# Ajax0564/VyomAI

Hardware: AMD Instinct MI355X
Metric: training tokens/sec (12L d=768 seq=512 GPT-style decoder, CLM) (higher is better)
Workload: dtype bf16; 1 GPU; configs[1]: GPT-style Decoder 12L d=768 h=12 RoPE vocab 50265, CLM training B=32/GPU seq=512, AdamW, bf16 kernels + fp32 masters; global_batch=32, seq_len=512, parallelism=dp1, attention=none, weights=deterministic recipe (vyomai_amd.recipe)

## Files before the change

### include/vyom_hip.h

```cpp
#ifndef VYOM_HIP_H
#define VYOM_HIP_H

#include <stdint.h>

#ifdef __cplusplus
extern "C" {
#endif

typedef enum { VY_F32 = 0, VY_BF16 = 1 } vy_dtype;

typedef enum {
  VY_OK = 0,
  VY_ERR_ARG = -1,
  VY_ERR_UNSUPPORTED = -2,
  VY_ERR_LAUNCH = -3
} vy_status;

typedef enum {
  VY_ACT_NONE = 0, VY_ACT_GELU_ERF = 1, VY_ACT_GELU_TANH = 2,
  VY_ACT_SILU = 3, VY_ACT_TANH = 4, VY_ACT_SIGMOID = 5, VY_ACT_RELU6 = 6, VY_ACT_LEAKY_RELU = 7
} vy_act;
#define VY_ACT_SAVE_DERIV 0x100

enum {
// ... 190 lines not shown
int vy_linear_dropout_fwd(const void* x, int64_t ldx, const void* w, int64_t ldw, const void* bias,
                          const void* residual, int64_t ldr, void* y, int64_t ldy, int64_t M, int64_t N,
                          int64_t K, float p_drop, uint64_t seed, uint64_t offset, int dtype, void* stream);
int vy_dropout(const void* x, int64_t ldx, void* y, int64_t ldy, int64_t M, int64_t N, float p_drop,
               uint64_t seed, uint64_t offset, int dtype, void* stream);

int vy_act_bwd(const void* dy, int64_t lddy, const void* pre, int64_t ldpre, void* dx, int64_t lddx,
               int64_t M, int64_t N, int act, int dtype, void* stream);

int vy_xent_fwd(const void* logits, int64_t ld, const int64_t* labels, int64_t ignore_index, float* lse,
                float* loss_sum, float* count, int64_t M, int64_t V, int32_t* err_flag, int dtype, void* stream);
int vy_xent_bwd(void* logits, int64_t ld, const int64_t* labels, int64_t ignore_index, const float* lse,
                const float* gscale, const float* count, int64_t M, int64_t V, int dtype, void* stream);
int vy_xent_fused(void* logits, int64_t ld, const int64_t* labels, int64_t ignore_index, float* lse,
                  float* loss_sum, const float* count, const float* gscale, int64_t M, int64_t V,
                  int32_t* err_flag, int dtype, void* stream);
int vy_xent_sample_fwd(const void* logits, int64_t ld, const int64_t* labels, int64_t ignore_index, float* lse,
                       float* loss_sum, float* count, int64_t* sampled, float inv_temperature, uint64_t seed,
                       uint64_t offset, int64_t M, int64_t V, int32_t* err_flag, int dtype, void* stream);
int vy_xent_sample_fused(void* logits, int64_t ld, const int64_t* labels, int64_t ignore_index, float* lse,
                         float* loss_sum, const float* count, const float* gscale, int64_t* sampled,
                         float inv_temperature, uint64_t seed, uint64_t offset, int64_t M, int64_t V,
                         int32_t* err_flag, int dtype, void* stream);
int vy_gumbel_noise(float* out, int64_t ld, int64_t M, int64_t V, uint64_t seed, uint64_t offset, void* stream);

int vy_bce_head_fwd(const void* h, int64_t ldh, const void* w, const void* b, float* z, const float* target,
                    const uint8_t* live, float* loss_sum, int64_t M, int64_t d, int dtype, void* stream);
int vy_bce_head_bwd(const void* h, int64_t ldh, const void* w, const float* z, const float* target,
                    const uint8_t* live, const float* gscale, const float* count, void* dh, int64_t lddh, float* dw,
                    float* db, int accumulate, int64_t M, int64_t d, int dtype, void* stream);

int vy_mlm_mask(const int64_t* ids, int64_t n, const int64_t* special_ids, int32_t n_special, float fraction,
                int64_t mask_id, int64_t vocab, int64_t ignore_index, uint64_t seed, uint64_t offset,
                int64_t* masked_ids, int64_t* labels, uint8_t* masked, void* stream);


int vy_logprob_fwd(const void* logits, int64_t ld, const int64_t* labels, const float* weight, float* lse,
                   float* logp, int64_t M, int64_t V, int32_t* err_flag, int dtype, void* stream);
int vy_logprob_bwd(void* logits, int64_t ld, const int64_t* labels, const float* weight, const float* lse,
                   int64_t M, int64_t V, int dtype, void* stream);
int vy_logprob_fused(void* logits, int64_t ld, const int64_t* labels, const float* weight, float* lse,
                     float* logp, int64_t M, int64_t V, int32_t* err_flag, int dtype, void* stream);

int vy_embedding_fwd(const void* table, int64_t ldt, const int64_t* ids, void* out, int64_t ldo,
                     int64_t M, int64_t d, int64_t V, int32_t* err_flag, int dtype, void* stream);
int vy_embedding_bwd(const void* dout, int64_t lddo, const int64_t* ids, float* dw, int64_t lddw,
// ... 126 lines not shown
```

### vyomai_amd/_lib.py

```python
from __future__ import annotations

import ctypes as C
import os
from typing import Optional

_HERE = os.path.dirname(os.path.abspath(__file__))
LIB_PATH = os.environ.get("VY_LIB_PATH") or os.path.join(_HERE, "lib", "libvyom_hip.so")

VY_F32, VY_BF16 = 0, 1
ACT_NONE, ACT_GELU_ERF, ACT_GELU_TANH = 0, 1, 2
ACT_SILU, ACT_TANH, ACT_SIGMOID, ACT_RELU6, ACT_LEAKY_RELU = 3, 4, 5, 6, 7
ACT_SAVE_DERIV = 0x100
LORA_EPI_ACT, LORA_EPI_DROP_RES, LORA_EPI_MUL = 0, 1, 2
MASK_NONE, MASK_CAUSAL, MASK_KEYPAD, MASK_ADDITIVE = 0, 1, 2, 4

_p, _i64, _i, _f, _u64 = C.c_void_p, C.c_int64, C.c_int, C.c_float, C.c_uint64

PROTOTYPES = {
    "vy_linear_fwd": [_p, _i64, _p, _i64, _p, _p, _i64, _p, _i64, _p, _i64, _i64, _i64, _i, _i, _p],
    "vy_qkv_rope_fwd": [_p, _i64, _p, _i64, _p, _p, _p, _i64,
                        _p, _i64, _i64, _i64, _p, _i64, _i64, _i64, _p, _i64, _i64, _i64,
                        _i64, _i64, _i64, _i, _i, _i, _i, _p],
    "vy_attn_fwd": [_p, _i64, _i64, _i64, _p, _i64, _i64, _i64, _p, _i64, _i64, _i64,
                    _p, _i64, _i64, _p, _i, _i64, _p, _i64, _p, _i64, _i64,
# ... 23 lines not shown
                           _i64, _i64, _i, _i, _i, _i, _p],
    "vy_qknorm_bwd": [_p, _i64, _p, _i64, _p, _p, _f, _p, _p, _f, _p, _i64, _i, _i, _i, _i, _p],
    "vy_rope_fwd": [_p, _i64, _i64, _i64, _p, _p, _i64, _i64, _i, _i64, _i, _i, _i, _p],
    "vy_linear_dgrad": [_p, _i64, _p, _i64, _p, _i64, _i, _p, _i64, _p, _i64, _p, _i64, _i64, _i64, _i64, _i, _p],
    "vy_linear_wgrad": [_p, _i64, _p, _i64, _p, _i64, _p, _f, _p, _i64, _i64, _i64, _i, _p],
    "vy_linear_wgrad_grouped": [_p, _i, _i, _p],
    "vy_linear_wgrad_grouped_cs": [_p, _i, _p, _i, _i, _p],
    "vy_linear_wgrad_grouped_opt": [_p, _i, _p, _i, _p, _i, _p, _i, _p],
    "vy_layernorm_bwd_partial": [_p, _i64, _p, _i64, _p, _p, _p, _p, _i64, _p, _i64, _i64, _i, _p],
    "vy_layernorm_bwd": [_p, _i64, _p, _i64, _p, _p, _p, _p, _i64, _p, _p, _f, _p, _i64, _i64, _i, _p],
    "vy_attn_bwd": [_p, _i64, _i64, _i64, _p, _i64, _i64, _i64, _p, _i64, _i64, _i64,
                    _p, _p, _i64, _i64, _p, _p,
                    _p, _i64, _i64, _i64, _p, _i64, _i64, _i64, _p, _i64, _i64, _i64,
                    _i, _i64, _p, _i64, _p, _p, _i64, _i64, _i, _i, _i64, _i64, _i, _f, _i, _p],
    "vy_adamw_step": [_p, _p, _p, _p, _p, _i64, _f, _f, _f, _f, _f, _i64, _f, _p, _p],
    "vy_adamw_step_gated": [_p, _p, _p, _p, _p, _i64, _f, _f, _f, _f, _f, _i64, _f, _p, _p, _p],
    "vy_sumsq": [_p, _i64, _p, _p, _p],
    "vy_linear_dropout_fwd": [_p, _i64, _p, _i64, _p, _p, _i64, _p, _i64, _i64, _i64, _i64, _f, _u64, _u64, _i, _p],
    "vy_dropout": [_p, _i64, _p, _i64, _i64, _i64, _f, _u64, _u64, _i, _p],
    "vy_act_bwd": [_p, _i64, _p, _i64, _p, _i64, _i64, _i64, _i, _i, _p],
    "vy_xent_fwd": [_p, _i64, _p, _i64, _p, _p, _p, _i64, _i64, _p, _i, _p],
    "vy_xent_bwd": [_p, _i64, _p, _i64, _p, _p, _p, _i64, _i64, _i, _p],
    "vy_xent_fused": [_p, _i64, _p, _i64, _p, _p, _p, _p, _i64, _i64, _p, _i, _p],
    "vy_xent_sample_fwd": [_p, _i64, _p, _i64, _p, _p, _p, _p, _f, _u64, _u64, _i64, _i64, _p, _i, _p],
    "vy_xent_sample_fused": [_p, _i64, _p, _i64, _p, _p, _p, _p, _p, _f, _u64, _u64, _i64, _i64, _p, _i, _p],
    "vy_gumbel_noise": [_p, _i64, _i64, _i64, _u64, _u64, _p],
    "vy_bce_head_fwd": [_p, _i64, _p, _p, _p, _p, _p, _p, _i64, _i64, _i, _p],
    "vy_bce_head_bwd": [_p, _i64, _p, _p, _p, _p, _p, _p, _p, _i64, _p, _p, _i, _i64, _i64, _i, _p],
    "vy_mlm_mask": [_p, _i64, _p, _i, _f, _i64, _i64, _i64, _u64, _u64, _p, _p, _p, _p],
    "vy_logprob_fwd": [_p, _i64, _p, _p, _p, _p, _i64, _i64, _p, _i, _p],
    "vy_logprob_bwd": [_p, _i64, _p, _p, _p, _i64, _i64, _i, _p],
    "vy_logprob_fused": [_p, _i64, _p, _p, _p, _p, _i64, _i64, _p, _i, _p],
    "vy_transpose_batched": [_p, _i, _i, _i, _p],
    "vy_embedding_fwd": [_p, _i64, _p, _p, _i64, _i64, _i64, _i64, _p, _i, _p],
    "vy_embedding_bwd": [_p, _i64, _p, _p, _i64, _i64, _i64, _i64, _i64, _i, _p],
    "vy_transpose": [_p, _i64, _p, _i64, _i64, _i64, _i, _p],
    "vy_greedy_step": [_p, _i64, _i64, _i64, _i, _p, _i64, _i64, _p, _i64, _p, _i, _p, _p, _p],
    "vy_sampling_probs": [_p, _i64, _i64, _i64, _i, _f, _i, _f, _p, _i64, _p],
    "vy_sample_rows": [_p, _i64, _i64, _i64, _i, _p, _p, _p, _p, _p, _p, _p],
    "vy_spec_verify": [_p, _i64, _i64, _p, _i64, _i64, _i64, _i64, _i64, _i, _p, _p, _p, _p, _p, _p, _p, _p, _p, _p, _p],
    "vy_lora_shrink": [_p, _i64, _p, _p, _i64, _p, _i64, _i64, _i64, _i64, _i64, _i, _p],
    "vy_lora_expand": [_p, _i64, _p, _i64, _p, _p, _p, _i64, _i64, _i64, _i64, _i64, _i64, _i64, _i, _p],
    "vy_lora_expand_epi": [_p, _i64, _p, _i64, _p, _i64, _p, _i64, _p, _i64, _p, _p, _p, _i64, _i64, _i64, _i64, _i64,
                           _i64, _i64, _i, _i, _f, _u64, _u64, _i, _p],
    "vy_cls_head_fwd": [_p, _i64, _p, _p, _p, _p, _p, _p, _p, _i64, _i64, _i64, _i, _p],
    "vy_cls_head_bwd": [_p, _i64, _p, _p, _p, _p, _p, _p, _i, _i64, _i64, _i64, _i64, _i, _p],
# ... 102 lines not shown
```

### vyomai_amd/autograd_train.py

```python
from __future__ import annotations

import os

import weakref
from typing import NamedTuple, Optional

import torch

from . import _lib, ops
from ._lib import ACT_GELU_ERF, ACT_NONE, VyomHipError
from .autograd import gated_mlp
from .layers.attention import _shadow
from .layers.mask import AttnMask
from .layers.positional_embeddings import resolve_freqs

BF16 = torch.bfloat16


WEIGHT_EPOCH = [0]


class _WtRegistry:

    def __init__(self) -> None:
# ... 581 lines not shown
    dt = n.dtype
    V = w.shape[0]
    ld = _row_stride(V)
    buf = torch.empty((n.numel() // n.shape[-1], ld), dtype=dt, device=n.device)
    if zero_pad and ld != V:
        buf[:, V:].zero_()
    logits = buf[:, :V]
    ops.linear(n.view(buf.shape[0], -1), _shadow(w, dt), None if bias is None else _shadow(bias, dt), out=logits)
    return buf, logits


def _rehome(x, ld, dtype, reuse=False):
    V = x.shape[-1]
    if reuse and x.stride(-1) == 1 and x.stride(-2) == ld and x.dtype == dtype:
        buf = torch.as_strided(x, (*x.shape[:-1], ld), x.stride())
        if ld != V:
            buf[..., V:].zero_()
        return buf
    buf = torch.zeros((*x.shape[:-1], ld), dtype=dtype, device=x.device)
    buf[..., :V] = x
    return buf


def _shifted_labels(labels, ignore_index, dev):
    shifted = torch.full(labels.shape, ignore_index, dtype=torch.long, device=dev)
    shifted[:, :-1] = labels[:, 1:]
    return shifted.view(-1)


def _xent_forward(logits, shifted, ignore_index, err_flag=None, in_place=True, sample=None):
    V = logits.shape[1]
    dev = logits.device
    lse = torch.empty(logits.shape[0], dtype=torch.float32, device=dev)
    acc = torch.zeros(2, dtype=torch.float32, device=dev)
    fused = in_place and V <= 65536 and logits.dtype == BF16
    if fused:
        acc[1] = ((shifted != ignore_index) & (shifted >= 0) & (shifted < V)).sum()
        if sample is None:
            ops.xent_fused_(logits, shifted, ignore_index, lse, acc[0:1], acc[1:2], _one(dev), err_flag)
        else:
            ops.xent_sample_fused_(logits, shifted, ignore_index, lse, acc[0:1], acc[1:2], _one(dev), *sample, err_flag)
    elif sample is None:
        ops.xent_fwd(logits, shifted, ignore_index, lse, acc[0:1], acc[1:2], err_flag)
    else:
        ops.xent_sample_fwd(logits, shifted, ignore_index, lse, acc[0:1], acc[1:2], *sample, err_flag)
    return acc[0] / acc[1].clamp_min(1.0), lse, acc, fused


def _xent_backward(logits, shifted, ignore_index, lse, acc, fused, gout):
    gs = gout.detach().to(torch.float32).reshape(1).contiguous()
    if fused:
        return gs
    ops.xent_bwd_(logits, shifted, ignore_index, lse, gs, acc[1:2])
    return None


class LMHeadFn(torch.autograd.Function):

    @staticmethod
    def forward(ctx, hidden, wd, bd, ln_w, ln_b, wv, bias, eps):
        _require_bf16(hidden)
        dt = hidden.dtype
        pre, g, n, mean, rstd = _head_transform(hidden, wd, bd, ln_w, ln_b, eps)
        V = wv.shape[0]
        ld = _row_stride(V)
        buf = torch.zeros((*hidden.shape[:-1], ld), dtype=dt, device=hidden.device)
        logits = buf[..., :V]
        ops.linear(n, _shadow(wv, dt), _shadow(bias, dt), out=logits)
        ctx.save_for_backward(hidden, pre, g, n, mean, rstd)
        ctx.params = (wd, bd, ln_w, ln_b, wv, bias)
        ctx.ld = ld
        return logits

    @staticmethod
    def backward(ctx, dlogits):
        hidden, pre, g, n, mean, rstd = ctx.saved_tensors
        wd, bd, ln_w, ln_b, wv, bias = ctx.params
        dt = hidden.dtype
        buf = _rehome(dlogits, ctx.ld, dt, reuse=True)
        dn = ops.linear_dgrad(buf, _wt_padded(wv, dt, ctx.ld))
        dwv, dbias = _wgrad(buf[..., :wv.shape[0]], n, wv, bias)
        return (*_head_transform_backward(dn, hidden, pre, g, mean, rstd, wd, bd, ln_w, ln_b), dwv, dbias, None)


class LMHeadLossFn(torch.autograd.Function):

    @staticmethod
    def forward(ctx, hidden, labels, ignore_index, wd, bd, ln_w, ln_b, wv, bias, eps, err_flag=None, shift=True,
                sample=None):
        _require_bf16(hidden)
        pre, g, n, mean, rstd = _head_transform(hidden, wd, bd, ln_w, ln_b, eps)
        buf, logits = _vocab_logits(n, wv, bias)
        dev = hidden.device
        shifted = _shifted_labels(labels, ignore_index, dev) if shift else labels.to(dev).reshape(-1).contiguous()
        sampled = None
        if sample is not None:
            sampled = torch.empty(shifted.shape, dtype=torch.long, device=dev)
            sample = (sampled, *sample)
        loss, lse, acc, fused = _xent_forward(logits, shifted, ignore_index, err_flag, sample=sample)
        ctx.save_for_backward(hidden, pre, g, n, mean, rstd, buf, shifted, lse, acc)
        ctx.params = (wd, bd, ln_w, ln_b, wv, bias)
        ctx.ignore = ignore_index
        ctx.fused = fused
        if sampled is None:
            return loss
        sampled = sampled.view(labels.shape)
        ctx.mark_non_differentiable(sampled)
        return loss, sampled

    @staticmethod
    def backward(ctx, gout, *_):
        hidden, pre, g, n, mean, rstd, buf, shifted, lse, acc = ctx.saved_tensors
        wd, bd, ln_w, ln_b, wv, bias = ctx.params
        dt = hidden.dtype
        logits = buf[:, :wv.shape[0]]
        alpha = _xent_backward(logits, shifted, ctx.ignore, lse, acc, ctx.fused, gout)
        dn = ops.linear_dgrad(buf, _wt_padded(wv, dt, buf.shape[1]))
        if alpha is not None:
            dn = dn * alpha.to(dt)
        dwv, dbias = _wgrad(logits, n.view(buf.shape[0], -1), wv, bias, alpha=alpha)
        dh, dwd, dbd, dgam, dbet = _head_transform_backward(dn.view(g.shape), hidden, pre, g, mean, rstd, wd, bd, ln_w, ln_b)
        return dh, None, None, dwd, dbd, dgam, dbet, dwv, dbias, None, None, None, None
# ... 393 lines not shown
        ctx.save_for_backward(n)
        ctx.meta = (table, table_pending, ld)
        return logits

    @staticmethod
    def backward(ctx, dlogits):
        (n,) = ctx.saved_tensors
        table, table_pending, ld = ctx.meta
        V = table.shape[0]
        buf = _rehome(dlogits.reshape(-1, V), ld, n.dtype)
        dn, dtab = _tied_head_backward(buf, V, n, table, table_pending, None)
        return dn, dtab, None


class ShiftedXentFn(torch.autograd.Function):

    @staticmethod
    def forward(ctx, logits, labels, ignore_index):
        _require_bf16(logits)
        B, L, V = logits.shape
        if logits.stride(-1) != 1 or logits.stride(1) % 8 or logits.stride(0) != L * logits.stride(1):
            logits = _rehome(logits, _row_stride(V), logits.dtype)[..., :V]
        l2 = torch.as_strided(logits, (B * L, V), (logits.stride(1), 1), logits.storage_offset())
        shifted = _shifted_labels(labels, ignore_index, logits.device)
        loss, lse, acc, _ = _xent_forward(l2, shifted, ignore_index, in_place=False)
        ctx.save_for_backward(l2, shifted, lse, acc)
        ctx.meta = (ignore_index, (B, L, V))
        return loss

    @staticmethod
    def backward(ctx, gout):
        l2, shifted, lse, acc = ctx.saved_tensors
        ignore_index, shape = ctx.meta
        ld = l2.stride(0)
        buf = torch.empty((l2.shape[0], ld), dtype=l2.dtype, device=l2.device)
        d2 = buf[:, :l2.shape[1]]
        d2.copy_(l2)
        _xent_backward(d2, shifted, ignore_index, lse, acc, False, gout)
        return torch.as_strided(buf, shape, (shape[1] * ld, ld, 1)), None, None


class TiedLMHeadLossFn(torch.autograd.Function):

    @staticmethod
    def forward(ctx, hidden, labels, ignore_index, ln_w, eps, table, table_pending, err_flag=None):
        _require_bf16(hidden)
        n = ops.rmsnorm(hidden, _shadow(ln_w, hidden.dtype), eps, 0.0)
        buf, logits = _vocab_logits(n, table, None)
        shifted = _shifted_labels(labels, ignore_index, hidden.device)
        loss, lse, acc, fused = _xent_forward(logits, shifted, ignore_index, err_flag)
        ctx.save_for_backward(hidden, n, buf, shifted, lse, acc)
        ctx.meta = (ln_w, eps, table, table_pending, ignore_index, fused)
        return loss

    @staticmethod
    def backward(ctx, gout):
        hidden, n, buf, shifted, lse, acc = ctx.saved_tensors
        ln_w, eps, table, table_pending, ignore_index, fused = ctx.meta
        V = table.shape[0]
        alpha = _xent_backward(buf[:, :V], shifted, ignore_index, lse, acc, fused, gout)
        dn, dtab = _tied_head_backward(buf, V, n, table, table_pending, alpha)
        dh, dlnw = _rms_bwd(dn, hidden, ln_w, eps)
        return dh, None, None, dlnw, None, dtab, None, None


def logprob_rows(input_ids, selection_mask):
    B, L = input_ids.shape
    labels = torch.zeros((B, L), dtype=torch.long, device=input_ids.device)
    labels[:, :-1] = input_ids[:, 1:]
    m = selection_mask.to(device=input_ids.device, dtype=torch.float32)
    w = torch.zeros((B, L), dtype=torch.float32, device=input_ids.device)
    w[:, :-1] = m[:, 1:]
    total = w.sum(-1, keepdim=True)
    w = torch.where(total > 0, w / total.clamp_min(torch.finfo(torch.float32).tiny), torch.zeros_like(w))
    return labels.view(-1), w


def tied_head_logprobs(hidden, labels, w, ln_w, eps, table, err_flag=None, in_place=False):
    dev = hidden.device
    n = ops.rmsnorm(hidden, _shadow(ln_w, hidden.dtype), eps, 0.0)
    buf, logits = _vocab_logits(n, table, None, zero_pad=in_place)
    wrow = w.reshape(-1)
    lse = torch.empty(buf.shape[0], dtype=torch.float32, device=dev)
    logp = torch.empty(buf.shape[0], dtype=torch.float32, device=dev)
    fused = in_place and table.shape[0] <= 65536 and hidden.dtype == BF16
    if fused:
        ops.logprob_fused_(logits, labels, wrow, lse, logp, err_flag)
    else:
        ops.logprob_fwd(logits, labels, wrow, lse, logp, err_flag)
    return (logp.view(w.shape) * w).sum(-1), (n, buf, wrow, lse, fused)


class TiedLMHeadLogprobFn(torch.autograd.Function):

    @staticmethod
    def forward(ctx, hidden, labels, w, ln_w, eps, table, table_pending, err_flag=None):
        _require_bf16(hidden)
        seq, (n, buf, wrow, lse, fused) = tied_head_logprobs(hidden, labels, w, ln_w, eps, table, err_flag, in_place=True)
        ctx.save_for_backward(hidden, n, buf, labels, wrow, lse)
        ctx.meta = (ln_w, eps, table, table_pending, fused, w.shape)
        return seq

    @staticmethod
    def backward(ctx, gseq):
        hidden, n, buf, labels, wrow, lse = ctx.saved_tensors
        ln_w, eps, table, table_pending, fused, (B, L) = ctx.meta
        V = table.shape[0]
        if not fused:
            ops.logprob_bwd_(buf[:, :V], labels, wrow, lse)
        g_row = gseq.detach().to(torch.float32).reshape(B, 1).expand(B, L).reshape(-1)
# ... 4 lines not shown
```

### vyomai_amd/csrc/vy_misc.hip

```cpp
#include "vy_common.h"
#include "vy_colsum.h"
#include <stdarg.h>
#include <string.h>

static thread_local char g_err[512] = "";
void vy_set_error(const char* fmt, ...) {
  va_list ap;
  va_start(ap, fmt);
  vsnprintf(g_err, sizeof(g_err), fmt, ap);
  va_end(ap);
}
extern "C" const char* vy_last_error(void) { return g_err; }
extern "C" int vy_abi_version(void) { return 5; }

namespace {

template <typename T, int CH>
__global__ __launch_bounds__(256) void layernorm_fwd_kernel(const T* __restrict__ x, int64_t ldx,
                                                            const T* __restrict__ gamma,
                                                            const T* __restrict__ beta, T* __restrict__ y,
                                                            int64_t ldy, float* __restrict__ mean_out,
                                                            float* __restrict__ rstd_out, int64_t M, int N,
                                                            float eps) {
  constexpr int VEC = Chunk<T>::VEC;
// ... 573 lines not shown
  const int64_t label = labels[m];
  T* row = logits + m * ld;
  const int nch = (V + VEC - 1) / VEC;
  const auto s = p.load(m, true);
  const bool dead = !p.live(s, label) || label < 0 || label >= V;
  const float l = lse[m];
  for (int c = threadIdx.x; c < nch; c += blockDim.x) {
    float v[VEC], o[VEC];
    Chunk<T>::load(row + (int64_t)c * VEC, v);
#pragma unroll
    for (int e = 0; e < VEC; ++e) {
      const int col = c * VEC + e;
      float g = 0.f;
      if (!dead && col < V) g = p.grad(s, __expf(v[e] - l), col == label ? 1.f : 0.f);
      o[e] = g;
    }
    Chunk<T>::store(row + (int64_t)c * VEC, o);
  }
}

template <typename P>
__global__ __launch_bounds__(1024) void row_fused_kernel(bf16* __restrict__ logits, int64_t ld,
                                                         const int64_t* __restrict__ labels, const P p,
                                                         float* __restrict__ lse, int V, int* __restrict__ err) {
  constexpr int CPT = 8;
  __shared__ float red[16];
  const int tid = threadIdx.x;
  const int64_t m = blockIdx.x;
  const int64_t label = labels[m];
  const auto s = p.load(m, true);
  bf16* row = logits + m * ld;
  const int nch = (V + 7) / 8;
  bf16x8 zero8;
#pragma unroll
  for (int e = 0; e < 8; ++e) zero8[e] = (bf16)0.f;
  const bool live = p.live(s, label);
  const bool oob = live && (label < 0 || label >= V);
  if (oob && err && tid == 0) *err = 1;
  if (!live || oob) {
    for (int c = tid; c < nch; c += 1024) *reinterpret_cast<bf16x8*>(row + (int64_t)c * 8) = zero8;
    if (tid == 0) { lse[m] = 0.f; p.skip(m); }
    return;
  }
  const float x_label = (float)row[label];
  bf16x8 v[CPT];
#pragma unroll
  for (int i = 0; i < CPT; ++i) {
    const int c = tid + i * 1024;
    if (c < nch) v[i] = *reinterpret_cast<const bf16x8*>(row + (int64_t)c * 8);
  }
  float mx = -INFINITY;
#pragma unroll
  for (int i = 0; i < CPT; ++i) {
    const int c = tid + i * 1024;
    if (c < nch) {
#pragma unroll
      for (int e = 0; e < 8; ++e)
        if (c * 8 + e < V) mx = fmaxf(mx, (float)v[i][e]);
    }
  }
  if constexpr (P::kSample) {
    __shared__ RowBest redb[16];
    RowBest best{-INFINITY, INT32_MAX};
#pragma unroll
    for (int i = 0; i < CPT; ++i) {
      const int c = tid + i * 1024;
      if (c < nch) {
        float f[8];
        Chunk<bf16>::unpack(v[i], f);
        p.template scan<8>(m, c, f, V, best);
      }
    }
    const RowBest g = block_argmax(best, redb);
// ... 11 lines not shown
    }
  }
  const float gsm = block_reduce(sm, red, false);
  const float l = gmx + __logf(gsm);
  if (tid == 0) {
    lse[m] = l;
    p.emit(m, l, x_label);
  }
#pragma unroll
  for (int i = 0; i < CPT; ++i) {
    const int c = tid + i * 1024;
    if (c < nch) {
      bf16x8 o;
#pragma unroll
      for (int e = 0; e < 8; ++e) {
        const int col = c * 8 + e;
        float g = 0.f;
        if (col < V) g = p.grad(s, __expf((float)v[i][e] - l), col == label ? 1.f : 0.f);
        o[e] = (bf16)g;
      }
      *reinterpret_cast<bf16x8*>(row + (int64_t)c * 8) = o;
    }
  }
}

int row_check(const char* fn, bool ptrs, const void* logits, int64_t ld, int64_t M, int64_t V, int dtype, const char* pair) {
  if (!ptrs || M <= 0 || V <= 0) VY_FAIL(VY_ERR_ARG, "%s: bad arguments", fn);
  if (pair) {
    if (dtype != VY_BF16) VY_FAIL(VY_ERR_UNSUPPORTED, "%s: bf16 only (use %s)", fn, pair);
    if (V > 65536) VY_FAIL(VY_ERR_UNSUPPORTED, "%s: V=%ld exceeds the 65536 columns a workgroup keeps in registers (use %s)", fn, (long)V, pair);
    if (ld % 8 || ld < vy_cdiv(V, 8) * 8 || (uintptr_t)logits % 16) VY_FAIL(VY_ERR_ARG, "%s: rows must be 16-byte aligned and cover the padded width", fn);
    return VY_OK;
  }
  const int vec = dtype == VY_BF16 ? 8 : 4;
  if (ld % vec || ld < vy_cdiv(V, vec) * vec) VY_FAIL(VY_ERR_ARG, "%s: row stride must be a multiple of %d and cover the padded row", fn, vec);
  if (dtype != VY_BF16 && dtype != VY_F32) VY_FAIL(VY_ERR_ARG, "%s: bad dtype %d", fn, dtype);
  return VY_OK;
}

template <typename P>
int row_lse(const char* fn, bool ptrs, const void* logits, int64_t ld, const int64_t* labels, const P& p, float* lse,
            int64_t M, int64_t V, int32_t* err, int dtype, void* stream) {
  if (const int rc = row_check(fn, ptrs && logits && labels && lse, logits, ld, M, V, dtype, nullptr)) return rc;
  const dim3 grid((unsigned)M), block(256);
  if (dtype == VY_BF16) hipLaunchKernelGGL((row_lse_kernel<bf16, P>), grid, block, 0, (hipStream_t)stream, (const bf16*)logits, ld, labels, p, lse, (int)V, err);
  else hipLaunchKernelGGL((row_lse_kernel<float, P>), grid, block, 0, (hipStream_t)stream, (const float*)logits, ld, labels, p, lse, (int)V, err);
  VY_CHECK_LAUNCH(fn);
  return VY_OK;
}

template <typename P>
int row_grad(const char* fn, bool ptrs, void* logits, int64_t ld, const int64_t* labels, const P& p, const float* lse,
             int64_t M, int64_t V, int dtype, void* stream) {
  if (const int rc = row_check(fn, ptrs && logits && labels && lse, logits, ld, M, V, dtype, nullptr)) return rc;
  const dim3 grid((unsigned)M), block(256);
  if (dtype == VY_BF16) hipLaunchKernelGGL((row_grad_kernel<bf16, P>), grid, block, 0, (hipStream_t)stream, (bf16*)logits, ld, labels, p, lse, (int)V);
  else hipLaunchKernelGGL((row_grad_kernel<float, P>), grid, block, 0, (hipStream_t)stream, (float*)logits, ld, labels, p, lse, (int)V);
  VY_CHECK_LAUNCH(fn);
  return VY_OK;
}

template <typename P>
int row_fused(const char* fn, bool ptrs, void* logits, int64_t ld, const int64_t* labels, const P& p, float* lse,
              int64_t M, int64_t V, int32_t* err, int dtype, void* stream) {
  if (const int rc = row_check(fn, ptrs && logits && labels && lse, logits, ld, M, V, dtype, P::kPair)) return rc;
  hipLaunchKernelGGL((row_fused_kernel<P>), dim3((unsigned)M), dim3(1024), 0, (hipStream_t)stream, (bf16*)logits, ld, labels, p, lse, (int)V, err);
  VY_CHECK_LAUNCH(fn);
  return VY_OK;
}

template <typename T>
int ln_fwd_dispatch(const void* x, int64_t ldx, const void* gamma, const void* beta, void* y, int64_t ldy,
                    float* mean, float* rstd, int64_t M, int64_t N, float eps, hipStream_t st) {
  constexpr int VEC = Chunk<T>::VEC;
  if (N % VEC || ldx % VEC || ldy % VEC) VY_FAIL(VY_ERR_ARG, "vy_layernorm_fwd: N/ld must be multiples of %d", VEC);
  const int nch = (int)(N / VEC);
  const dim3 grid((unsigned)vy_cdiv(M, 4)), block(256);
#define LN_GO(CH)                                                                                       \
  hipLaunchKernelGGL((layernorm_fwd_kernel<T, CH>), grid, block, 0, st, (const T*)x, ldx, (const T*)gamma, \
                     (const T*)beta, (T*)y, ldy, mean, rstd, M, (int)N, eps)
  if (nch <= 64) LN_GO(1);
  else if (nch <= 128) LN_GO(2);
  else if (nch <= 256) LN_GO(4);
  else if (nch <= 512) LN_GO(8);
  else if (nch <= 1024) LN_GO(16);
  else VY_FAIL(VY_ERR_UNSUPPORTED, "vy_layernorm_fwd: N=%ld too wide", (long)N);
#undef LN_GO
  VY_CHECK_LAUNCH("vy_layernorm_fwd");
  return VY_OK;
// ... 221 lines not shown
                                    int32_t* err_flag, int dtype, void* stream) {
  XentSampleRow<false> p{{ignore_index, gscale, count, loss_sum, nullptr}, sampled, inv_temperature, vy_make_noise(seed, offset)};
  return row_fused("vy_xent_sample_fused", loss_sum && count && gscale && sampled, logits, ld, labels, p, lse, M, V, err_flag, dtype, stream);
}

extern "C" int vy_logprob_fwd(const void* logits, int64_t ld, const int64_t* labels, const float* weight, float* lse,
                              float* logp, int64_t M, int64_t V, int32_t* err_flag, int dtype, void* stream) {
  return row_lse("vy_logprob_fwd", weight && logp, logits, ld, labels, LogprobRow{weight, logp}, lse, M, V, err_flag,
                 dtype, stream);
}

extern "C" int vy_logprob_bwd(void* logits, int64_t ld, const int64_t* labels, const float* weight, const float* lse,
                              int64_t M, int64_t V, int dtype, void* stream) {
  return row_grad("vy_logprob_bwd", weight != nullptr, logits, ld, labels, LogprobRow{weight, nullptr}, lse, M, V, dtype,
                  stream);
}

extern "C" int vy_logprob_fused(void* logits, int64_t ld, const int64_t* labels, const float* weight, float* lse,
                                float* logp, int64_t M, int64_t V, int32_t* err_flag, int dtype, void* stream) {
  return row_fused("vy_logprob_fused", weight && logp, logits, ld, labels, LogprobRow{weight, logp}, lse, M, V,
                   err_flag, dtype, stream);
}

extern "C" int vy_cast(const void* src, void* dst, int64_t n, int src_dtype, int dst_dtype, void* stream) {
  if (!src || !dst || n < 0) VY_FAIL(VY_ERR_ARG, "vy_cast: bad arguments");
  if (n == 0) return VY_OK;
  hipStream_t st = (hipStream_t)stream;
  const int64_t want = vy_cdiv(n, 1024);
  const dim3 grid((unsigned)(want < 4096 ? want : 4096)), block(256);
  if (src_dtype == VY_F32 && dst_dtype == VY_BF16)
    hipLaunchKernelGGL((cast_kernel<float, bf16>), grid, block, 0, st, (const float*)src, (bf16*)dst, n);
  else if (src_dtype == VY_BF16 && dst_dtype == VY_F32)
    hipLaunchKernelGGL((cast_kernel<bf16, float>), grid, block, 0, st, (const bf16*)src, (float*)dst, n);
  else VY_FAIL(VY_ERR_ARG, "vy_cast: unsupported %d -> %d", src_dtype, dst_dtype);
  VY_CHECK_LAUNCH("vy_cast");
  return VY_OK;
}

template <typename T>
__global__ __launch_bounds__(256) void embedding_fwd_kernel(const T* __restrict__ table, int64_t ldt,
                                                            const int64_t* __restrict__ ids, T* __restrict__ out,
                                                            int64_t ldo, int64_t M, int d, int64_t V, int* err) {
  constexpr int VEC = Chunk<T>::VEC;
  const int lane = threadIdx.x & 63;
  const int64_t m = (int64_t)blockIdx.x * 4 + (threadIdx.x >> 6);
  if (m >= M) return;
// ... 254 lines not shown
```

### vyomai_amd/ops.py

```python
from __future__ import annotations

import math
from typing import NamedTuple, Optional, Sequence, Tuple

import torch

from . import _lib
from ._lib import call, dtype_code

Tensor = torch.Tensor




class _Lanes:
    active = False
    side: Optional[torch.cuda.Stream] = None
    fork_ev: Optional[torch.cuda.Event] = None
    join_ev: Optional[torch.cuda.Event] = None
    B = L = B0 = 0
    dirty = False
    keep: list = []
    streams = {}

# ... 489 lines not shown
        host = torch.from_numpy(np.frombuffer(bytes(arr), dtype=np.uint8).copy())
        self.table = host.to(pairs[0][0].device)

    def run(self) -> None:
        call("vy_transpose_batched", self.table.data_ptr(), self.n, self.total, dtype_code(self.dtype), _stream())


def cast(src: Tensor, dst: Tensor) -> Tensor:
    _need_gpu(src, dst)
    call("vy_cast", src.data_ptr(), dst.data_ptr(), src.numel(), dtype_code(src.dtype), dtype_code(dst.dtype), _stream())
    return dst


def act_bwd(dy: Tensor, pre: Tensor, act: int) -> Tensor:
    _need_gpu(dy, pre)
    d2, p2 = _rows(dy), _rows(pre)
    M, N = p2.shape
    out = torch.empty((M, N), dtype=dy.dtype, device=dy.device)
    call("vy_act_bwd", d2.data_ptr(), d2.stride(0), p2.data_ptr(), p2.stride(0), out.data_ptr(), out.stride(0),
         M, N, act, dtype_code(dy.dtype), _stream())
    return out.view(pre.shape)


def _row_args(logits2d: Tensor, labels: Tensor, *rows: Tensor, scalars=()) -> None:
    M = logits2d.shape[0]
    assert labels.dtype == torch.long and labels.numel() == M and labels.is_contiguous()
    for t in rows:
        assert t.dtype == torch.float32 and t.numel() == M and t.is_contiguous()
    for t in scalars:
        assert t.dtype == torch.float32 and t.numel() == 1


def xent_fwd(logits2d: Tensor, labels: Tensor, ignore_index: int, lse: Tensor, loss_sum: Tensor, count: Tensor,
             err_flag: Optional[Tensor] = None) -> None:
    _need_gpu(logits2d, labels, lse, loss_sum, count, err_flag)
    _row_args(logits2d, labels, lse, scalars=(loss_sum, count))
    M, V = logits2d.shape
    call("vy_xent_fwd", logits2d.data_ptr(), logits2d.stride(0), labels.data_ptr(), ignore_index, lse.data_ptr(),
         loss_sum.data_ptr(), count.data_ptr(), M, V, _ptr(err_flag), dtype_code(logits2d.dtype), _stream())


def xent_bwd_(logits2d: Tensor, labels: Tensor, ignore_index: int, lse: Tensor, gscale: Tensor, count: Tensor) -> None:
    _need_gpu(logits2d, labels, lse, gscale, count)
    _row_args(logits2d, labels, lse, scalars=(gscale, count))
    M, V = logits2d.shape
    call("vy_xent_bwd", logits2d.data_ptr(), logits2d.stride(0), labels.data_ptr(), ignore_index, lse.data_ptr(),
         gscale.data_ptr(), count.data_ptr(), M, V, dtype_code(logits2d.dtype), _stream())


def xent_fused_(logits2d: Tensor, labels: Tensor, ignore_index: int, lse: Tensor, loss_sum: Tensor,
                count: Tensor, gscale: Tensor, err_flag: Optional[Tensor] = None) -> None:
    _need_gpu(logits2d, labels, lse, loss_sum, count, gscale, err_flag)
    _row_args(logits2d, labels, lse, scalars=(loss_sum, count, gscale))
    M, V = logits2d.shape
    call("vy_xent_fused", logits2d.data_ptr(), logits2d.stride(0), labels.data_ptr(), ignore_index, lse.data_ptr(),
         loss_sum.data_ptr(), count.data_ptr(), gscale.data_ptr(), M, V, _ptr(err_flag), dtype_code(logits2d.dtype),
         _stream())


def xent_sample_fwd(logits2d: Tensor, labels: Tensor, ignore_index: int, lse: Tensor, loss_sum: Tensor, count: Tensor,
                    sampled: Tensor, inv_temperature: float, seed: int, offset: int,
                    err_flag: Optional[Tensor] = None) -> None:
    _need_gpu(logits2d, labels, lse, loss_sum, count, sampled, err_flag)
    _row_args(logits2d, labels, lse, scalars=(loss_sum, count))
    M, V = logits2d.shape
    assert sampled.dtype == torch.long and sampled.numel() == M and sampled.is_contiguous()
    call("vy_xent_sample_fwd", logits2d.data_ptr(), logits2d.stride(0), labels.data_ptr(), ignore_index, lse.data_ptr(),
         loss_sum.data_ptr(), count.data_ptr(), sampled.data_ptr(), float(inv_temperature), int(seed), int(offset), M, V,
         _ptr(err_flag), dtype_code(logits2d.dtype), _stream())


def xent_sample_fused_(logits2d: Tensor, labels: Tensor, ignore_index: int, lse: Tensor, loss_sum: Tensor, count: Tensor,
                       gscale: Tensor, sampled: Tensor, inv_temperature: float, seed: int, offset: int,
                       err_flag: Optional[Tensor] = None) -> None:
    _need_gpu(logits2d, labels, lse, loss_sum, count, gscale, sampled, err_flag)
    _row_args(logits2d, labels, lse, scalars=(loss_sum, count, gscale))
    M, V = logits2d.shape
    assert sampled.dtype == torch.long and sampled.numel() == M and sampled.is_contiguous()
    call("vy_xent_sample_fused", logits2d.data_ptr(), logits2d.stride(0), labels.data_ptr(), ignore_index,
         lse.data_ptr(), loss_sum.data_ptr(), count.data_ptr(), gscale.data_ptr(), sampled.data_ptr(),
         float(inv_temperature), int(seed), int(offset), M, V, _ptr(err_flag), dtype_code(logits2d.dtype), _stream())


def gumbel_noise(M: int, V: int, seed: int, offset: int, device) -> Tensor:
    out = torch.empty((M, V), dtype=torch.float32, device=device)
    _need_gpu(out)
    call("vy_gumbel_noise", out.data_ptr(), out.stride(0), M, V, int(seed), int(offset), _stream())
    return out


def _bce_args(h2: Tensor, w: Tensor, M: int, *rows: Tensor, scalars=()) -> None:
    assert w.dtype == h2.dtype and w.numel() == h2.shape[1] and w.is_contiguous()
    for t in rows:
        assert t.numel() == M and t.is_contiguous()
    for t in scalars:
        assert t.dtype == torch.float32 and t.numel() == 1


def bce_head_fwd(h: Tensor, w: Tensor, b: Optional[Tensor], target: Optional[Tensor] = None,
                 live: Optional[Tensor] = None, loss_sum: Optional[Tensor] = None) -> Tensor:
    _need_gpu(h, w, b, target, live, loss_sum)
    h2 = _rows(h)
# ... 539 lines not shown
    call("vy_embedding_bwd", d2.data_ptr(), d2.stride(0), idc.data_ptr(), dw.data_ptr(), dw.stride(0),
         -1 if padding_idx is None else int(padding_idx), d2.shape[0], d2.shape[1], dw.shape[0],
         dtype_code(dout.dtype), _stream())


def logprob_fwd(logits2d: Tensor, labels: Tensor, weight: Tensor, lse: Tensor, logp: Tensor,
                err_flag: Optional[Tensor] = None) -> None:
    _need_gpu(logits2d, labels, weight, lse, logp, err_flag)
    _row_args(logits2d, labels, weight, lse, logp)
    M, V = logits2d.shape
    call("vy_logprob_fwd", logits2d.data_ptr(), logits2d.stride(0), labels.data_ptr(), weight.data_ptr(), lse.data_ptr(),
         logp.data_ptr(), M, V, _ptr(err_flag), dtype_code(logits2d.dtype), _stream())


def logprob_bwd_(logits2d: Tensor, labels: Tensor, weight: Tensor, lse: Tensor) -> None:
    _need_gpu(logits2d, labels, weight, lse)
    _row_args(logits2d, labels, weight, lse)
    M, V = logits2d.shape
    call("vy_logprob_bwd", logits2d.data_ptr(), logits2d.stride(0), labels.data_ptr(), weight.data_ptr(), lse.data_ptr(),
         M, V, dtype_code(logits2d.dtype), _stream())


def logprob_fused_(logits2d: Tensor, labels: Tensor, weight: Tensor, lse: Tensor, logp: Tensor,
                   err_flag: Optional[Tensor] = None) -> None:
    _need_gpu(logits2d, labels, weight, lse, logp, err_flag)
    _row_args(logits2d, labels, weight, lse, logp)
    M, V = logits2d.shape
    call("vy_logprob_fused", logits2d.data_ptr(), logits2d.stride(0), labels.data_ptr(), weight.data_ptr(),
         lse.data_ptr(), logp.data_ptr(), M, V, _ptr(err_flag), dtype_code(logits2d.dtype), _stream())


def rmsnorm(x: Tensor, w: Tensor, eps: float, w_offset: float = 1.0) -> Tensor:
    _need_gpu(x, w)
    x2 = _rows(x)
    M, N = x2.shape
    y = torch.empty((M, N), dtype=x.dtype, device=x.device)
    call("vy_rmsnorm_fwd", x2.data_ptr(), x2.stride(0), w.data_ptr(), y.data_ptr(), y.stride(0), M, N, float(eps),
         float(w_offset), dtype_code(x.dtype), _stream())
    return y.view(x.shape)


def gated_act(gate_up: Tensor, act: int) -> Tensor:
    _need_gpu(gate_up)
    g2 = _rows(gate_up)
    M, two_i = g2.shape
    I = two_i // 2
    out = torch.empty((M, I), dtype=gate_up.dtype, device=gate_up.device)
    call("vy_gated_act_fwd", g2.data_ptr(), g2.stride(0), out.data_ptr(), out.stride(0), M, I, act,
         dtype_code(gate_up.dtype), _stream())
    return out.view(*gate_up.shape[:-1], I)

# ... 223 lines not shown
```

Measured before the change: 908,500 tokens/s.

## Fuse CLM label shift and count, zero logit padding inside fused xent kernel

```diff
diff --git a/include/vyom_hip.h b/include/vyom_hip.h
--- a/include/vyom_hip.h
+++ b/include/vyom_hip.h
@@ -236,6 +236,17 @@
                          float* loss_sum, const float* count, const float* gscale, int64_t* sampled,
                          float inv_temperature, uint64_t seed, uint64_t offset, int64_t M, int64_t V,
                          int32_t* err_flag, int dtype, void* stream);
+int vy_xent_fused_padded(void* logits, int64_t ld, const int64_t* labels, int64_t ignore_index, float* lse,
+                         float* loss_sum, const float* count, const float* gscale, int64_t M, int64_t V,
+                         int32_t* err_flag, int dtype, void* stream);
+int vy_xent_sample_fused_padded(void* logits, int64_t ld, const int64_t* labels, int64_t ignore_index, float* lse,
+                                float* loss_sum, const float* count, const float* gscale, int64_t* sampled,
+                                float inv_temperature, uint64_t seed, uint64_t offset, int64_t M, int64_t V,
+                                int32_t* err_flag, int dtype, void* stream);
+int vy_logprob_fused_padded(void* logits, int64_t ld, const int64_t* labels, const float* weight, float* lse,
+                            float* logp, int64_t M, int64_t V, int32_t* err_flag, int dtype, void* stream);
+int vy_clm_targets(const int64_t* labels, int64_t* targets, float* acc, int64_t B, int64_t L, int64_t ignore_index,
+                   int64_t V, int shift, void* stream);
 int vy_gumbel_noise(float* out, int64_t ld, int64_t M, int64_t V, uint64_t seed, uint64_t offset, void* stream);
 
 int vy_bce_head_fwd(const void* h, int64_t ldh, const void* w, const void* b, float* z, const float* target,
diff --git a/vyomai_amd/_lib.py b/vyomai_amd/_lib.py
--- a/vyomai_amd/_lib.py
+++ b/vyomai_amd/_lib.py
@@ -69,6 +69,10 @@
     "vy_xent_fwd": [_p, _i64, _p, _i64, _p, _p, _p, _i64, _i64, _p, _i, _p],
     "vy_xent_bwd": [_p, _i64, _p, _i64, _p, _p, _p, _i64, _i64, _i, _p],
     "vy_xent_fused": [_p, _i64, _p, _i64, _p, _p, _p, _p, _i64, _i64, _p, _i, _p],
+    "vy_xent_fused_padded": [_p, _i64, _p, _i64, _p, _p, _p, _p, _i64, _i64, _p, _i, _p],
+    "vy_xent_sample_fused_padded": [_p, _i64, _p, _i64, _p, _p, _p, _p, _p, _f, _u64, _u64, _i64, _i64, _p, _i, _p],
+    "vy_logprob_fused_padded": [_p, _i64, _p, _p, _p, _p, _i64, _i64, _p, _i, _p],
+    "vy_clm_targets": [_p, _p, _p, _i64, _i64, _i64, _i64, _i, _p],
     "vy_xent_sample_fwd": [_p, _i64, _p, _i64, _p, _p, _p, _p, _f, _u64, _u64, _i64, _i64, _p, _i, _p],
     "vy_xent_sample_fused": [_p, _i64, _p, _i64, _p, _p, _p, _p, _p, _f, _u64, _u64, _i64, _i64, _p, _i, _p],
     "vy_gumbel_noise": [_p, _i64, _i64, _i64, _u64, _u64, _p],
diff --git a/vyomai_amd/autograd_train.py b/vyomai_amd/autograd_train.py
--- a/vyomai_amd/autograd_train.py
+++ b/vyomai_amd/autograd_train.py
@@ -627,28 +627,31 @@
     return buf
 
 
-def _shifted_labels(labels, ignore_index, dev):
-    shifted = torch.full(labels.shape, ignore_index, dtype=torch.long, device=dev)
-    shifted[:, :-1] = labels[:, 1:]
-    return shifted.view(-1)
-
-
-def _xent_forward(logits, shifted, ignore_index, err_flag=None, in_place=True, sample=None):
+def _fused_rows(V, dtype, in_place=True):
+    return in_place and V <= 65536 and dtype == BF16
+
+
+def _targets(labels, ignore_index, V, dev, shift=True):
+    return ops.clm_targets(labels.to(dev).reshape(-1, labels.shape[-1]), ignore_index, V, shift)
+
+
+def _xent_forward(logits, shifted, ignore_index, acc, err_flag=None, in_place=True, sample=None):
     V = logits.shape[1]
     dev = logits.device
     lse = torch.empty(logits.shape[0], dtype=torch.float32, device=dev)
-    acc = torch.zeros(2, dtype=torch.float32, device=dev)
-    fused = in_place and V <= 65536 and logits.dtype == BF16
+    fused = _fused_rows(V, logits.dtype, in_place)
     if fused:
-        acc[1] = ((shifted != ignore_index) & (shifted >= 0) & (shifted < V)).sum()
         if sample is None:
-            ops.xent_fused_(logits, shifted, ignore_index, lse, acc[0:1], acc[1:2], _one(dev), err_flag)
+            ops.xent_fused_(logits, shifted, ignore_index, lse, acc[0:1], acc[1:2], _one(dev), err_flag, zero_pad=True)
         else:
-            ops.xent_sample_fused_(logits, shifted, ignore_index, lse, acc[0:1], acc[1:2], _one(dev), *sample, err_flag)
-    elif sample is None:
-        ops.xent_fwd(logits, shifted, ignore_index, lse, acc[0:1], acc[1:2], err_flag)
+            ops.xent_sample_fused_(logits, shifted, ignore_index, lse, acc[0:1], acc[1:2], _one(dev), *sample, err_flag,
+                                   zero_pad=True)
     else:
-        ops.xent_sample_fwd(logits, shifted, ignore_index, lse, acc[0:1], acc[1:2], *sample, err_flag)
+        acc[1:2].zero_()
+        if sample is None:
+            ops.xent_fwd(logits, shifted, ignore_index, lse, acc[0:1], acc[1:2], err_flag)
+        else:
+            ops.xent_sample_fwd(logits, shifted, ignore_index, lse, acc[0:1], acc[1:2], *sample, err_flag)
     return acc[0] / acc[1].clamp_min(1.0), lse, acc, fused
 
 
@@ -695,14 +698,14 @@
                 sample=None):
         _require_bf16(hidden)
         pre, g, n, mean, rstd = _head_transform(hidden, wd, bd, ln_w, ln_b, eps)
-        buf, logits = _vocab_logits(n, wv, bias)
+        buf, logits = _vocab_logits(n, wv, bias, zero_pad=not _fused_rows(wv.shape[0], n.dtype))
         dev = hidden.device
-        shifted = _shifted_labels(labels, ignore_index, dev) if shift else labels.to(dev).reshape(-1).contiguous()
+        shifted, acc = _targets(labels, ignore_index, wv.shape[0], dev, shift)
         sampled = None
         if sample is not None:
             sampled = torch.empty(shifted.shape, dtype=torch.long, device=dev)
             sample = (sampled, *sample)
-        loss, lse, acc, fused = _xent_forward(logits, shifted, ignore_index, err_flag, sample=sample)
+        loss, lse, acc, fused = _xent_forward(logits, shifted, ignore_index, acc, err_flag, sample=sample)
         ctx.save_for_backward(hidden, pre, g, n, mean, rstd, buf, shifted, lse, acc)
         ctx.params = (wd, bd, ln_w, ln_b, wv, bias)
         ctx.ignore = ignore_index
@@ -1142,8 +1145,8 @@
         if logits.stride(-1) != 1 or logits.stride(1) % 8 or logits.stride(0) != L * logits.stride(1):
             logits = _rehome(logits, _row_stride(V), logits.dtype)[..., :V]
         l2 = torch.as_strided(logits, (B * L, V), (logits.stride(1), 1), logits.storage_offset())
-        shifted = _shifted_labels(labels, ignore_index, logits.device)
-        loss, lse, acc, _ = _xent_forward(l2, shifted, ignore_index, in_place=False)
+        shifted, acc = _targets(labels, ignore_index, V, logits.device)
+        loss, lse, acc, _ = _xent_forward(l2, shifted, ignore_index, acc, in_place=False)
         ctx.save_for_backward(l2, shifted, lse, acc)
         ctx.meta = (ignore_index, (B, L, V))
         return loss
@@ -1166,9 +1169,9 @@
     def forward(ctx, hidden, labels, ignore_index, ln_w, eps, table, table_pending, err_flag=None):
         _require_bf16(hidden)
         n = ops.rmsnorm(hidden, _shadow(ln_w, hidden.dtype), eps, 0.0)
-        buf, logits = _vocab_logits(n, table, None)
-        shifted = _shifted_labels(labels, ignore_index, hidden.device)
-        loss, lse, acc, fused = _xent_forward(logits, shifted, ignore_index, err_flag)
+        buf, logits = _vocab_logits(n, table, None, zero_pad=not _fused_rows(table.shape[0], n.dtype))
+        shifted, acc = _targets(labels, ignore_index, table.shape[0], hidden.device)
+        loss, lse, acc, fused = _xent_forward(logits, shifted, ignore_index, acc, err_flag)
         ctx.save_for_backward(hidden, n, buf, shifted, lse, acc)
         ctx.meta = (ln_w, eps, table, table_pending, ignore_index, fused)
         return loss
@@ -1199,13 +1202,13 @@
 def tied_head_logprobs(hidden, labels, w, ln_w, eps, table, err_flag=None, in_place=False):
     dev = hidden.device
     n = ops.rmsnorm(hidden, _shadow(ln_w, hidden.dtype), eps, 0.0)
-    buf, logits = _vocab_logits(n, table, None, zero_pad=in_place)
+    fused = _fused_rows(table.shape[0], hidden.dtype, in_place)
+    buf, logits = _vocab_logits(n, table, None, zero_pad=in_place and not fused)
     wrow = w.reshape(-1)
     lse = torch.empty(buf.shape[0], dtype=torch.float32, device=dev)
     logp = torch.empty(buf.shape[0], dtype=torch.float32, device=dev)
-    fused = in_place and table.shape[0] <= 65536 and hidden.dtype == BF16
     if fused:
-        ops.logprob_fused_(logits, labels, wrow, lse, logp, err_flag)
+        ops.logprob_fused_(logits, labels, wrow, lse, logp, err_flag, zero_pad=True)
     else:
         ops.logprob_fwd(logits, labels, wrow, lse, logp, err_flag)
     return (logp.view(w.shape) * w).sum(-1), (n, buf, wrow, lse, fused)
diff --git a/vyomai_amd/csrc/vy_misc.hip b/vyomai_amd/csrc/vy_misc.hip
--- a/vyomai_amd/csrc/vy_misc.hip
+++ b/vyomai_amd/csrc/vy_misc.hip
@@ -619,15 +619,23 @@
 template <typename P>
 __global__ __launch_bounds__(1024) void row_fused_kernel(bf16* __restrict__ logits, int64_t ld,
                                                          const int64_t* __restrict__ labels, const P p,
-                                                         float* __restrict__ lse, int V, int* __restrict__ err) {
+                                                         float* __restrict__ lse, int V, int width,
+                                                         int* __restrict__ err) {
   constexpr int CPT = 8;
   __shared__ float red[16];
   const int tid = threadIdx.x;
   const int64_t m = blockIdx.x;
+  bf16* row = logits + m * ld;
+  const int nch = (V + 7) / 8;
+  bf16x8 v[CPT];
+#pragma unroll
+  for (int i = 0; i < CPT; ++i) {
+    const int c = tid + i * 1024;
+    v[i] = *reinterpret_cast<const bf16x8*>(row + (int64_t)(c < nch ? c : nch - 1) * 8);
+  }
+  __builtin_amdgcn_sched_barrier(0);
   const int64_t label = labels[m];
   const auto s = p.load(m, true);
-  bf16* row = logits + m * ld;
-  const int nch = (V + 7) / 8;
   bf16x8 zero8;
 #pragma unroll
   for (int e = 0; e < 8; ++e) zero8[e] = (bf16)0.f;
@@ -635,17 +643,11 @@
   const bool oob = live && (label < 0 || label >= V);
   if (oob && err && tid == 0) *err = 1;
   if (!live || oob) {
-    for (int c = tid; c < nch; c += 1024) *reinterpret_cast<bf16x8*>(row + (int64_t)c * 8) = zero8;
+    for (int c = tid; c < width / 8; c += 1024) *reinterpret_cast<bf16x8*>(row + (int64_t)c * 8) = zero8;
     if (tid == 0) { lse[m] = 0.f; p.skip(m); }
     return;
   }
   const float x_label = (float)row[label];
-  bf16x8 v[CPT];
-#pragma unroll
-  for (int i = 0; i < CPT; ++i) {
-    const int c = tid + i * 1024;
-    if (c < nch) v[i] = *reinterpret_cast<const bf16x8*>(row + (int64_t)c * 8);
-  }
   float mx = -INFINITY;
 #pragma unroll
   for (int i = 0; i < CPT; ++i) {
@@ -703,6 +705,7 @@
       *reinterpret_cast<bf16x8*>(row + (int64_t)c * 8) = o;
     }
   }
+  for (int c = nch + tid; c < width / 8; c += 1024) *reinterpret_cast<bf16x8*>(row + (int64_t)c * 8) = zero8;
 }
 
 int row_check(const char* fn, bool ptrs, const void* logits, int64_t ld, int64_t M, int64_t V, int dtype, const char* pair) {
@@ -743,9 +746,11 @@
 
 template <typename P>
 int row_fused(const char* fn, bool ptrs, void* logits, int64_t ld, const int64_t* labels, const P& p, float* lse,
-              int64_t M, int64_t V, int32_t* err, int dtype, void* stream) {
+              int64_t M, int64_t V, int32_t* err, int dtype, void* stream, bool pad = false) {
   if (const int rc = row_check(fn, ptrs && logits && labels && lse, logits, ld, M, V, dtype, P::kPair)) return rc;
-  hipLaunchKernelGGL((row_fused_kernel<P>), dim3((unsigned)M), dim3(1024), 0, (hipStream_t)stream, (bf16*)logits, ld, labels, p, lse, (int)V, err);
+  if (pad && ld > INT32_MAX) VY_FAIL(VY_ERR_ARG, "%s: row stride %ld too wide to be a padded row", fn, (long)ld);
+  const int width = pad ? (int)ld : (int)(vy_cdiv(V, 8) * 8);
+  hipLaunchKernelGGL((row_fused_kernel<P>), dim3((unsigned)M), dim3(1024), 0, (hipStream_t)stream, (bf16*)logits, ld, labels, p, lse, (int)V, width, err);
   VY_CHECK_LAUNCH(fn);
   return VY_OK;
 }
@@ -1013,6 +1018,79 @@
                    err_flag, dtype, stream);
 }
 
+extern "C" int vy_xent_fused_padded(void* logits, int64_t ld, const int64_t* labels, int64_t ignore_index, float* lse,
+                                    float* loss_sum, const float* count, const float* gscale, int64_t M, int64_t V,
+                                    int32_t* err_flag, int dtype, void* stream) {
+  return row_fused("vy_xent_fused_padded", loss_sum && count && gscale, logits, ld, labels,
+                   XentRow<false>{ignore_index, gscale, count, loss_sum, nullptr}, lse, M, V, err_flag, dtype, stream, true);
+}
+
+extern "C" int vy_xent_sample_fused_padded(void* logits, int64_t ld, const int64_t* labels, int64_t ignore_index,
+                                           float* lse, float* loss_sum, const float* count, const float* gscale,
+                                           int64_t* sampled, float inv_temperature, uint64_t seed, uint64_t offset,
+                                           int64_t M, int64_t V, int32_t* err_flag, int dtype, void* stream) {
+  XentSampleRow<false> p{{ignore_index, gscale, count, loss_sum, nullptr}, sampled, inv_temperature, vy_make_noise(seed, offset)};
+  return row_fused("vy_xent_sample_fused_padded", loss_sum && count && gscale && sampled, logits, ld, labels, p, lse, M, V,
+                   err_flag, dtype, stream, true);
+}
+
+extern "C" int vy_logprob_fused_padded(void* logits, int64_t ld, const int64_t* labels, const float* weight, float* lse,
+                                       float* logp, int64_t M, int64_t V, int32_t* err_flag, int dtype, void* stream) {
+  return row_fused("vy_logprob_fused_padded", weight && logp, logits, ld, labels, LogprobRow{weight, logp}, lse, M, V,
+                   err_flag, dtype, stream, true);
+}
+
+namespace {
+__global__ __launch_bounds__(1024) void clm_targets_kernel(const int64_t* __restrict__ labels, int64_t* __restrict__ targets,
+                                                           float* __restrict__ acc, int64_t B, int64_t L, int64_t ignore,
+                                                           int64_t V, int shift) {
+  __shared__ unsigned long long red[16];
+  const int64_t n = B * L;
+  unsigned long long cnt = 0;
+  constexpr int U = 16;
+  for (int64_t base = 0; base < n; base += 1024 * U) {
+    int64_t t[U];
+#pragma unroll
+    for (int k = 0; k < U; ++k) {
+      const int64_t i = base + k * 1024 + threadIdx.x;
+      t[k] = ignore;
+      if (i < n) {
+        const bool last = n <= UINT32_MAX ? (uint32_t)i % (uint32_t)L == (uint32_t)L - 1 : i % L == L - 1;
+        if (!shift) t[k] = labels[i];
+        else if (!last) t[k] = labels[i + 1];
+      }
+    }
+#pragma unroll
+    for (int k = 0; k < U; ++k) {
+      const int64_t i = base + k * 1024 + threadIdx.x;
+      if (i < n) {
+        targets[i] = t[k];
+        cnt += (t[k] != ignore && t[k] >= 0 && t[k] < V) ? 1u : 0u;
+      }
+    }
+  }
+#pragma unroll
+  for (int o = 32; o > 0; o >>= 1) cnt += __shfl_xor(cnt, o, 64);
+  if ((threadIdx.x & 63) == 0) red[threadIdx.x >> 6] = cnt;
+  __syncthreads();
+  if (threadIdx.x == 0) {
+    unsigned long long total = 0;
+    for (int w = 0; w < 16; ++w) total += red[w];
+    acc[0] = 0.f;
+    acc[1] = (float)(long long)total;
+  }
+}
+}
+
+extern "C" int vy_clm_targets(const int64_t* labels, int64_t* targets, float* acc, int64_t B, int64_t L,
+                              int64_t ignore_index, int64_t V, int shift, void* stream) {
+  if (!labels || !targets || !acc || B <= 0 || L <= 0 || V <= 0) VY_FAIL(VY_ERR_ARG, "vy_clm_targets: bad arguments");
+  hipLaunchKernelGGL(clm_targets_kernel, dim3(1), dim3(1024), 0, (hipStream_t)stream, labels, targets, acc, B, L,
+                     ignore_index, V, shift);
+  VY_CHECK_LAUNCH("vy_clm_targets");
+  return VY_OK;
+}
+
 extern "C" int vy_cast(const void* src, void* dst, int64_t n, int src_dtype, int dst_dtype, void* stream) {
   if (!src || !dst || n < 0) VY_FAIL(VY_ERR_ARG, "vy_cast: bad arguments");
   if (n == 0) return VY_OK;
diff --git a/vyomai_amd/ops.py b/vyomai_amd/ops.py
--- a/vyomai_amd/ops.py
+++ b/vyomai_amd/ops.py
@@ -535,6 +535,18 @@
     return out.view(pre.shape)
 
 
+def clm_targets(labels: Tensor, ignore_index: int, V: int, shift: bool) -> tuple:
+    _need_gpu(labels)
+    assert labels.dtype == torch.long and labels.dim() == 2
+    labels = labels.contiguous()
+    B, L = labels.shape
+    targets = torch.empty((B * L,), dtype=torch.long, device=labels.device)
+    acc = torch.empty((2,), dtype=torch.float32, device=labels.device)
+    call("vy_clm_targets", labels.data_ptr(), targets.data_ptr(), acc.data_ptr(), B, L, int(ignore_index), int(V),
+         1 if shift else 0, _stream())
+    return targets, acc
+
+
 def _row_args(logits2d: Tensor, labels: Tensor, *rows: Tensor, scalars=()) -> None:
     M = logits2d.shape[0]
     assert labels.dtype == torch.long and labels.numel() == M and labels.is_contiguous()
@@ -562,11 +574,11 @@
 
 
 def xent_fused_(logits2d: Tensor, labels: Tensor, ignore_index: int, lse: Tensor, loss_sum: Tensor,
-                count: Tensor, gscale: Tensor, err_flag: Optional[Tensor] = None) -> None:
+                count: Tensor, gscale: Tensor, err_flag: Optional[Tensor] = None, zero_pad: bool = False) -> None:
     _need_gpu(logits2d, labels, lse, loss_sum, count, gscale, err_flag)
     _row_args(logits2d, labels, lse, scalars=(loss_sum, count, gscale))
     M, V = logits2d.shape
-    call("vy_xent_fused", logits2d.data_ptr(), logits2d.stride(0), labels.data_ptr(), ignore_index, lse.data_ptr(),
+    call("vy_xent_fused_padded" if zero_pad else "vy_xent_fused", logits2d.data_ptr(), logits2d.stride(0), labels.data_ptr(), ignore_index, lse.data_ptr(),
          loss_sum.data_ptr(), count.data_ptr(), gscale.data_ptr(), M, V, _ptr(err_flag), dtype_code(logits2d.dtype),
          _stream())
 
@@ -585,12 +597,12 @@
 
 def xent_sample_fused_(logits2d: Tensor, labels: Tensor, ignore_index: int, lse: Tensor, loss_sum: Tensor, count: Tensor,
                        gscale: Tensor, sampled: Tensor, inv_temperature: float, seed: int, offset: int,
-                       err_flag: Optional[Tensor] = None) -> None:
+                       err_flag: Optional[Tensor] = None, zero_pad: bool = False) -> None:
     _need_gpu(logits2d, labels, lse, loss_sum, count, gscale, sampled, err_flag)
     _row_args(logits2d, labels, lse, scalars=(loss_sum, count, gscale))
     M, V = logits2d.shape
     assert sampled.dtype == torch.long and sampled.numel() == M and sampled.is_contiguous()
-    call("vy_xent_sample_fused", logits2d.data_ptr(), logits2d.stride(0), labels.data_ptr(), ignore_index,
+    call("vy_xent_sample_fused_padded" if zero_pad else "vy_xent_sample_fused", logits2d.data_ptr(), logits2d.stride(0), labels.data_ptr(), ignore_index,
          lse.data_ptr(), loss_sum.data_ptr(), count.data_ptr(), gscale.data_ptr(), sampled.data_ptr(),
          float(inv_temperature), int(seed), int(offset), M, V, _ptr(err_flag), dtype_code(logits2d.dtype), _stream())
 
@@ -1176,11 +1188,11 @@
 
 
 def logprob_fused_(logits2d: Tensor, labels: Tensor, weight: Tensor, lse: Tensor, logp: Tensor,
-                   err_flag: Optional[Tensor] = None) -> None:
+                   err_flag: Optional[Tensor] = None, zero_pad: bool = False) -> None:
     _need_gpu(logits2d, labels, weight, lse, logp, err_flag)
     _row_args(logits2d, labels, weight, lse, logp)
     M, V = logits2d.shape
-    call("vy_logprob_fused", logits2d.data_ptr(), logits2d.stride(0), labels.data_ptr(), weight.data_ptr(),
+    call("vy_logprob_fused_padded" if zero_pad else "vy_logprob_fused", logits2d.data_ptr(), logits2d.stride(0), labels.data_ptr(), weight.data_ptr(),
          lse.data_ptr(), logp.data_ptr(), M, V, _ptr(err_flag), dtype_code(logits2d.dtype), _stream())
 
 
```

Result: no change. 909,800 tokens/s (median of 3 runs) (+0.1%).
